# artiom-matvei/RLAO

Measured on AMD Instinct MI355X. Metric: AO env-steps/sec (batched loops), higher is better.
Workload: dtype f32; 1 GPU; 8m / 20x20 Shack-Hartmann, 256 batched envs per GPU, integrator closed loop (BASELINE.json configs[1]); envs_per_gpu=256, envs_total=256, resolution=120, n_valid_act=357, n_signal=632, layers=1, controller=leaky integrator, gain 0.5, noise=photon, parallelism=env-shards x1, all-gather of episode returns

## Files before the change

include/aoenv.h:

```cpp
#ifndef AOENV_H
#define AOENV_H

#include <stddef.h>
#include <stdint.h>

#ifdef __cplusplus
extern "C" {
#endif

#define AOENV_ABI_VERSION 7

enum { AOENV_F32 = 0, AOENV_F64 = 1 };
enum { AOENV_WFS_SH = 0, AOENV_WFS_PYRAMID = 1 };

typedef struct AoEnv AoEnv;

typedef struct AoCfg {
    int32_t abi_version;
    int32_t dtype;
    int32_t n_env;
    int32_t resolution;
    int32_t n_layer;
    int32_t layer_res;
    int32_t n_inner;
// ... 213 lines not shown
int aoenv_set_detector(AoEnv* env, const AoDetector* cfg, void* stream);

int aoenv_set_return_accumulator(AoEnv* env, void* d_return);

int aoenv_buffer(AoEnv* env, int which, void** d_ptr, size_t* bytes);
int aoenv_download(AoEnv* env, int which, void* h_dst, size_t bytes, void* stream);
int aoenv_upload_state(AoEnv* env, int which, const void* h_src, size_t bytes, void* stream);
int aoenv_get_buff(AoEnv* env, double* h_buff);
int aoenv_set_buff(AoEnv* env, const double* h_buff);

enum AoOption {
    AOENV_OPT_FAST_WFS = 0,
    AOENV_OPT_MFMA_GEMM = 1,
    AOENV_OPT_STORE_ATM_OPD = 3,
    AOENV_OPT_FUSED_TAIL = 4,
    AOENV_OPT_FUSED_STEP = 5,
    AOENV_OPT_DEFER_RING = 6,
    AOENV_OPT_COEFS_IMAGE = 7,
    AOENV_OPT_FACTORED_RECON = 8,
    AOENV_OPT_RING_LOOKAHEAD = 9,
    AOENV_OPT_FAST_TRIG = 2,
    AOENV_OPT_ENV_WIND_PIXELS = 10,
    AOENV_OPT_STEP_PAIRS = 11,
    AOENV_OPT_FORCE_PATH = 99
};
enum AoPath {
    AOENV_PATH_PHASE_DWORD = 256,
    AOENV_PATH_GENERIC = 512,
    AOENV_PATH_PYR_ROUND_ROBIN = 1024,
    AOENV_PATH_MODAL_GEMM = 2048,
    AOENV_PATH_WF_GENERAL = 8192,
    AOENV_PATH_SCI_GENERAL = 16384,
    AOENV_PATH_SH_PLAIN = 4096
};
int aoenv_set_option(AoEnv* env, int option, int value);

int aoenv_fused_step_active(AoEnv* env);

enum AoKernel {
    AOENV_K_SHIFT_GATHER = 0, AOENV_K_MT_NORMAL, AOENV_K_GEMM_RING, AOENV_K_SCATTER, AOENV_K_PHASE,
    AOENV_K_SH_SPOTS, AOENV_K_SH_CENTROID, AOENV_K_GEMM_RECON, AOENV_K_RECON_FINISH, AOENV_K_PYRAMID, AOENV_K_SH_TAIL, AOENV_K_ENV_STEP,
    AOENV_K_DETECTOR, AOENV_K_COUNT
};
int aoenv_profile(AoEnv* env, int enable);
int aoenv_profile_read(AoEnv* env, double* h_ms, int32_t* h_count, void* stream);
int aoenv_step_counters(AoEnv* env, int64_t* h_out);

int aoenv_test_normal(int device, uint32_t seed, int n, int n_calls, double* h_out);

int aoenv_test_poisson_table(uint32_t* h_out, size_t cap_words, size_t* h_words);
int aoenv_test_poisson(int device, const float* h_lambda, int n, uint64_t seed, uint32_t frame, float lmax, float* h_out);

#ifdef __cplusplus
}
#endif
#endif
```

rlao_amd/_lib.py:

```python
from __future__ import annotations

import ctypes as C
import os

_HERE = os.path.dirname(os.path.abspath(__file__))
LIB_PATH = os.environ.get("AOENV_LIB") or os.path.join(_HERE, "csrc", "libaoenv.so")

ABI_VERSION = 7
F32, F64 = 0, 1
WFS_SH, WFS_PYRAMID = 0, 1

(C_PUPIL, C_AB, C_INNER_IDX, C_OUTER_IDX, C_LAYER_WEIGHT, C_DM_GX, C_DM_GY, C_DM_MODES, C_ACT_IDX, C_WFS_AMP,
 C_SH_SUBAP_IDX, C_SH_REF, C_WFS_UNITS, C_RECON, C_PYR_MASK, C_PYR_TT, C_RECON_FACTORS) = range(17)
(B_SCREEN, B_OPD_ATM, B_COEFS, B_PHASE, B_FRAME, B_SIGNAL, B_TOTAL, B_RESIDUAL, B_WFS_MAX, B_XI, B_MT_STATE,
 B_COUNTERS, B_DM_PREV, B_COEFS_SEEN) = range(14)


(OPT_FAST_WFS, OPT_MFMA_GEMM, OPT_FAST_TRIG, OPT_STORE_ATM_OPD, OPT_FUSED_TAIL, OPT_FUSED_STEP, OPT_DEFER_RING, OPT_COEFS_IMAGE,
 OPT_FACTORED_RECON, OPT_RING_LOOKAHEAD, OPT_ENV_WIND_PIXELS, OPT_STEP_PAIRS) = range(12)
OPT_FORCE_PATH = 99
MAX_DELAY = 8
PATH_PHASE_DWORD, PATH_GENERIC, PATH_PYR_ROUND_ROBIN, PATH_MODAL_GEMM, PATH_SH_PLAIN, PATH_WF_GENERAL = 256, 512, 1024, 2048, 4096, 8192
PATH_SCI_GENERAL = 16384
SCI_LOG10 = 1
WF_RESIDUAL, WF_ATMOSPHERE = 1, 2
MAX_WF_MODES = 1024
KERNEL_NAMES = ("ring_prepare", "mt_normal", "gemm_ring", "ring_scatter", "phase", "sh_spots", "sh_centroid",
                "gemm_recon", "recon_finish", "pyramid", "sh_tail", "env_step", "detector")


class AoCfg(C.Structure):
    _fields_ = [(n, C.c_int32) for n in (
        "abi_version", "dtype", "n_env", "resolution", "n_layer", "layer_res", "n_inner", "n_outer", "n_act",
        "n_valid_act", "dm_separable", "wfs_type", "n_subap", "n_valid_subap", "n_signal", "cam_res", "n_loop",
        "max_group", "pyr_n_res", "pyr_n_theta", "pyr_centering", "pyr_norm_valid", "pyr_q_lo", "pyr_q_hi")] + [
            ("layer_res_l", C.c_int32 * 8)] + [(n, C.c_double) for n in (
            "atm_wavelength", "src_wavelength", "leak", "threshold_cog")]


class AoDetector(C.Structure):
    _fields_ = [("photon_noise", C.c_int32), ("bits", C.c_int32), ("emccd", C.c_int32), ("env_index_offset", C.c_int32),
                ("qe", C.c_double), ("dark_electrons", C.c_double), ("fwc", C.c_double), ("gain", C.c_double),
# ... 80 lines not shown
    "aoenv_policy_forward": (C.c_int, [C.c_void_p, C.c_void_p, C.c_void_p, C.c_void_p, C.c_void_p, C.c_void_p]),
    "aoenv_run_policy_rollout": (C.c_int, [C.c_void_p, C.POINTER(AoRollout), C.c_void_p, C.c_void_p, C.c_void_p, C.c_void_p, C.c_void_p,
                                           C.c_void_p, C.c_void_p, C.c_void_p]),
    "aoenv_compute_psf": (C.c_int, [C.c_void_p, C.c_int, C.c_void_p, C.c_void_p]),
    "aoenv_set_science": (C.c_int, [C.c_void_p, C.POINTER(AoScience), C.c_void_p]),
    "aoenv_science_psf": (C.c_int, [C.c_void_p, C.c_int, C.c_void_p, C.c_void_p]),
    "aoenv_set_science_accumulator": (C.c_int, [C.c_void_p, C.c_void_p, C.c_void_p, C.c_void_p]),
    "aoenv_set_detector": (C.c_int, [C.c_void_p, C.c_void_p, C.c_void_p]),
    "aoenv_set_return_accumulator": (C.c_int, [C.c_void_p, C.c_void_p]),
    "aoenv_buffer": (C.c_int, [C.c_void_p, C.c_int, C.POINTER(C.c_void_p), C.POINTER(C.c_size_t)]),
    "aoenv_download": (C.c_int, [C.c_void_p, C.c_int, C.c_void_p, C.c_size_t, C.c_void_p]),
    "aoenv_upload_state": (C.c_int, [C.c_void_p, C.c_int, C.c_void_p, C.c_size_t, C.c_void_p]),
    "aoenv_set_wind_env": (C.c_int, [C.c_void_p, C.c_void_p, C.c_int, C.c_void_p]),
    "aoenv_get_clock_env": (C.c_int, [C.c_void_p, C.c_void_p]),
    "aoenv_set_clock_env": (C.c_int, [C.c_void_p, C.c_void_p]),
    "aoenv_set_r0_env": (C.c_int, [C.c_void_p, C.c_void_p, C.c_double, C.c_void_p]),
    "aoenv_get_r0_env": (C.c_int, [C.c_void_p, C.c_void_p]),
    "aoenv_get_buff": (C.c_int, [C.c_void_p, C.c_void_p]),
    "aoenv_set_buff": (C.c_int, [C.c_void_p, C.c_void_p]),
    "aoenv_set_option": (C.c_int, [C.c_void_p, C.c_int, C.c_int]),
    "aoenv_profile": (C.c_int, [C.c_void_p, C.c_int]),
    "aoenv_profile_read": (C.c_int, [C.c_void_p, C.c_void_p, C.c_void_p, C.c_void_p]),
    "aoenv_step_counters": (C.c_int, [C.c_void_p, C.c_void_p]),
    "aoenv_test_normal": (C.c_int, [C.c_int, C.c_uint32, C.c_int, C.c_int, C.c_void_p]),
    "aoenv_test_poisson_table": (C.c_int, [C.c_void_p, C.c_size_t, C.POINTER(C.c_size_t)]),
    "aoenv_test_poisson": (C.c_int, [C.c_int, C.c_void_p, C.c_int, C.c_uint64, C.c_uint32, C.c_float, C.c_void_p]),
}


class AoEnvError(RuntimeError):
    pass


_lib = None


def load():
    global _lib
    if _lib is not None:
        return _lib
    if not os.path.exists(LIB_PATH):
        raise AoEnvError(f"{LIB_PATH} not found: build it with `python -c 'import __graft_entry__ as g; g.build()'` "
                         "(there is no CPU fallback)")
    import torch
    lib = C.CDLL(LIB_PATH)
    for name, (res, args) in EXPORTS.items():
        if name == "aoenv_step_counters" and os.environ.get("AOENV_LIB") and not hasattr(lib, name):
            continue
        fn = getattr(lib, name)
        fn.restype = res
        fn.argtypes = args
    if lib.aoenv_abi_version() != ABI_VERSION:
        raise AoEnvError(f"libaoenv ABI {lib.aoenv_abi_version()} != binding ABI {ABI_VERSION}")
    _lib = lib
    return lib


def check(rc: int):
    if rc != 0:
        raise AoEnvError(load().aoenv_last_error().decode("utf-8", "replace"))
```

rlao_amd/csrc/camera_sh6.hpp:

```cpp
#pragma once
#include "detector.hpp"
#include "sh_device.hpp"

namespace ao {

typedef float f32x16s __attribute__((ext_vector_type(16)));

__device__ inline f32x16s camera_pack(const float (&Ia)[6], const float (&Ib)[6]) {
    return f32x16s{Ia[0], Ia[1], Ia[2], Ia[3], Ib[0], Ib[1], Ib[2], Ib[3], Ia[4], Ia[5], Ib[4], Ib[5], 0.f, 0.f, 0.f, 0.f};
}
__device__ inline void camera_unpack(const f32x16s& v, float (&Ia)[6], float (&Ib)[6]) {
    Ia[0] = v[0]; Ia[1] = v[1]; Ia[2] = v[2]; Ia[3] = v[3]; Ib[0] = v[4]; Ib[1] = v[5]; Ib[2] = v[6]; Ib[3] = v[7];
    Ia[4] = v[8]; Ia[5] = v[9]; Ib[4] = v[10]; Ib[5] = v[11];
}
__device__ inline void camera_rotate(f32x16s& v) {
    v = f32x16s{v[4], v[5], v[6], v[7], v[8], v[9], v[10], v[11], v[0], v[1], v[2], v[3], 0.f, 0.f, 0.f, 0.f};
}

template <bool PHOTON_ONLY = false>
__device__ inline void camera_sh6_lane(f32x16s& pxv, bool ok, uint32_t px0, int cam, uint32_t e, const DetectorCfg& det,
                                       const uint32_t* __restrict__ tab, float lmax) {
    auto pix_of = [&](int p) {
        const int t = p >> 2, s4 = p & 3;
        return px0 + (uint32_t)((t < 2 ? s4 : 4 + (s4 & 1)) * cam + ((t == 1 || (t == 2 && s4 >= 2)) ? 3 : 0));
// ... 63 lines not shown
                                                      : poisson_ptrs(det.dark_e, word_of(o, sl4), word_of(o2, sl4), pix_of(4 * t + sl4) | 0x80000000u, e, det);
            }
            if (has_read) {
                uint32_t o[4];
                quad_bits(qid, e, det, kDrawReadout, o);
                quad_normals(o, nrm);
            }
#pragma unroll
            for (int sl4 = 0; sl4 < 4; ++sl4) pxv[sl4] = detector_finish(pxv[sl4], det, dark[sl4], nrm[sl4]);
            camera_rotate(pxv);
        }
    }
}

typedef __attribute__((address_space(1))) const void* ao_gptr_t;
typedef __attribute__((address_space(3))) void* ao_lptr_t;
__device__ inline void alias_table_to_lds(const uint32_t* __restrict__ tab, int words, uint32_t* lds, int wave, int n_waves, int lane) {
    for (int i0 = wave * 256; i0 < words; i0 += n_waves * 256) {
        const int i = i0 + 4 * lane;
        if (i < words) __builtin_amdgcn_global_load_lds((ao_gptr_t)(tab + i), (ao_lptr_t)(lds + i0), 16, 0, 0);
    }
}

}
```

rlao_amd/csrc/common.hpp:

```cpp
#pragma once
#include <hip/hip_runtime.h>
#include <stdint.h>
#include <stddef.h>

#include <string>
#include <vector>

#include "aoenv.h"

namespace ao {

constexpr int kWave = 64;
constexpr int kMaxLayer = 8;
constexpr int kMtN = 624;
constexpr int kMaxSplits = 16;
constexpr int kMaxModes = 512;

int fail(const char* fmt, ...);
#define AO_HIP(call)                                                                          \
    do {                                                                                      \
        hipError_t e_ = (call);                                                               \
        if (e_ != hipSuccess)                                                                 \
            return ::ao::fail("%s:%d: %s -> %s", __FILE__, __LINE__, #call, hipGetErrorString(e_)); \
    } while (0)
// ... 283 lines not shown
    float* wfs_max;
    const float* fac_m;
    const float* fac_m2c_t;
    const short* slot_of;
    const float* amp_pupil;
    const float* gxa;
    const float* gya;
    size_t ga_env;
    DetectorCfg det;
    PoissonAlias pa;
    const float* ring_x[kMaxLayer];
    int ring_splits[kMaxLayer];
    const int* outer_idx;
    int n_outer;
    float* next_zx[kMaxLayer];
    int next_sx[kMaxLayer], next_sy[kMaxLayer];
    const int* inner_idx;
    int n_inner, zx_ld;
    int n_modes, n_subap, n_valid, n_env;
    LayerTaps taps2[kMaxLayer];
};
int step_fused_supported(int R, int n_subap, int n_valid, int n_act, int n_modes);
int step_alias_capacity(int n_act);
int launch_env_step(const StepArgs& a, const StarEnv<float>& star, hipStream_t st);
bool env_step_pairable(const StepArgs& a, const StarEnv<float>& star);
int launch_env_step_pair(const StepArgs& a, hipStream_t st);

template <typename T>
struct RolloutActionArgs {
    const T* obs;
    T* action;
    const T* fr;
    const T* fl_t;
    const int* act_slot;
    const T* sigma_env;
    T gain, sigma;
    int n_act, n_valid_act, n_filter;
    uint32_t seed_lo, seed_hi, counter, env_offset;
};
constexpr size_t kRolloutLdsMax = 160 * 1024;
size_t rollout_action_lds(int n_valid_act, int n_filter, size_t esz);
template <typename T>
int launch_rollout_action(const RolloutActionArgs<T>& a, int n_env, hipStream_t st);

template <typename T>
struct DisturbArgs {
    const T* coefs;
    T* seen;
    const T* modes_t;
// ... 141 lines not shown
```

rlao_amd/csrc/env.hip:

```cpp
#include <algorithm>
#include <cmath>
#include <cstdarg>
#include <cstdio>
#include <cstring>
#include <initializer_list>
#include <new>
#include <utility>

#include "common.hpp"
#include "delay.hpp"
#include "dev_block.hpp"
#include "dm_tables.hpp"
#include "detector.hpp"
#include "disturb.hpp"
#include "modal.hpp"
#include "policy.hpp"
#include "sh_device.hpp"
#include "science.hpp"
#include "star_env.hpp"
#include "wavefront.hpp"

namespace ao {

static thread_local std::string g_err;
// ... 216 lines not shown
    bool act_slot_dirty = true;
    void* rollout_scratch = nullptr;
    uint32_t explore_counter = 0;
    uint64_t explore_seed = 0;
    bool explore_seeded = false;
    struct Policy {
        bool set = false, mfma = false;
        Block mem;
        int H = 0, F = 0, Kp = 0;
        double slope = 0, clamp_abs = 0, b3 = 0;
        void *w1 = nullptr, *b1 = nullptr, *w2 = nullptr, *b2 = nullptr, *w3 = nullptr, *wt1 = nullptr, *wt2 = nullptr;
        void *proj_fr = nullptr, *proj_fl_t = nullptr, *hid1 = nullptr, *hid2 = nullptr;
    } policy;
    std::vector<Block> allocs;
    bool use_fast_wfs = true;
    bool use_mfma = true;
    bool use_fast_trig = true;
    bool use_fused_tail = true;
    bool use_fused_step = true;
    bool store_opd_atm = false;
    bool atm_user_defined = false;
    int force_path = 0;
    bool use_step_pairs = true;
    struct StepPair { bool on = false; double buff2[kMaxLayer][2] = {}; } pair;
    int64_t step_launches = 0, step_covered = 0;
    bool prof_on = false;
    struct ProfEv { int stage; hipEvent_t a, b; int n; };
    std::vector<ProfEv> prof_ev;

    template <typename T> T* as(void* p_) const { return static_cast<T*>(p_); }
    void* screen_ptr(int l) const { return static_cast<char*>(screen) + layer[l].scr_off * esz; }
    void* minmax_ptr(int l) const { return static_cast<char*>(minmax) + (size_t)l * E * 2 * esz; }
    void* xbuf_ptr(int l) const { return static_cast<char*>(xbuf) + (size_t)l * kMaxSplits * E * noutmax * esz; }
    void* zx_pipe_ptr(int buf, int l) const { return static_cast<char*>(zx_pipe) + ((size_t)buf * L + l) * E * Kmax * esz; }
};

namespace {

int dmalloc(AoEnv* env, void** p, size_t bytes, bool zero = true);
static int alloc_dm_rows(AoEnv* env) {
    if (env->esz == 4 && env->nAct <= 128) {
        if (!env->dm_rows)
            AO_TRY(dmalloc(env, (void**)&env->dm_rows, (size_t)env->E * (cdiv(env->R, 128) * 128) * 4 * env->ga_stride * sizeof(float)));
    } else if (!env->coefs_img) {
        AO_TRY(dmalloc(env, &env->coefs_img, (size_t)env->E * env->nAct * env->nAct * env->esz));
    }
// ... 601 lines not shown
    if (env->det.active) env->det.frame_counter += 1;
    a.det = env->det;
    a.pa = env->alias();
    take_rings(env, a);
    const Layer& y0 = env->layer[0];
    a.outer_idx = y0.outer_idx;
    a.n_outer = y0.nout;
    a.inner_idx = y0.inner_idx;
    a.n_inner = y0.nin;
    a.zx_ld = y0.K;
    a.n_modes = env->n_modes;
    a.n_subap = env->nSub;
    a.n_valid = env->nVal;
    a.n_env = env->E;
    const bool pair = env->pair.on;
    if (pair) {
        for (int l = 0; l < env->L; ++l) {
            a.taps2[l] = a.k.pa.taps[l];
            taps_from_buff(env->pair.buff2[l], a.taps2[l]);
        }
    }
    {
        AO_PROF_N(env, ENV_STEP, st, pair ? 2 : 1);
        AO_TRY(pair ? launch_env_step_pair(a, st) : launch_env_step(a, env->star_env<float>(), st));
    }
    env->step_launches += 1;
    env->step_covered += pair ? 2 : 1;
    rings_written(env);
    if (pair) {
        for (int l = 0; l < env->L; ++l) {
            LayerClock& c = env->layer[l].clk;
            if (c.ratio[0] == 0 && c.ratio[1] == 0) continue;
            int bx, by;
            if (clock_rounds(c.ratio, 0, &bx, &by) > 0 || clock_subpixel(c.ratio, c.buff, &bx, &by))
                return fail("internal: a step covered by the launch before it crossed a pixel");
        }
        if (env->det.active) env->det.frame_counter += 1;
    }
    return 0;
}

bool step_pair_eligible(AoEnv* env) {
    if (!env->use_step_pairs || env->esz != 4 || !fused_step_ok<float>(env) || env->per_env_wind) return false;
    if (env->disturb.set || env->wf.recorded() || env->store_opd_atm) return false;
    StepArgs a{};
    a.sc = sh_const<float>(env);
    a.det = env->det;
// ... 2220 lines not shown
    if (env->per_env_wind) return fail("the shard runs per-env clocks (aoenv_set_wind_env): use aoenv_set_clock_env");
    for (int l = 0; l < env->L; ++l) {
        if (std::fabs(h_buff[2 * l]) >= 1 || std::fabs(h_buff[2 * l + 1]) >= 1) return fail("|buff| must be < 1");
        env->layer[l].clk.buff[0] = h_buff[2 * l]; env->layer[l].clk.buff[1] = h_buff[2 * l + 1];
    }
    return 0;
}

int aoenv_fused_step_active(AoEnv* env) {
    if (!env) return 0;
    return env->c.dtype == AOENV_F32 && fused_step_ok<float>(env) ? 1 : 0;
}

int aoenv_set_option(AoEnv* env, int option, int value) {
    AO_CHECK_ENV(env);
    switch (option) {
        case AOENV_OPT_FAST_WFS: env->use_fast_wfs = value != 0; return 0;
        case AOENV_OPT_MFMA_GEMM: env->use_mfma = value != 0; return 0;
        case AOENV_OPT_FAST_TRIG: env->use_fast_trig = value != 0; return 0;
        case AOENV_OPT_STORE_ATM_OPD: env->store_opd_atm = value != 0; return 0;
        case AOENV_OPT_FUSED_TAIL: env->use_fused_tail = value != 0; return 0;
        case AOENV_OPT_FUSED_STEP: env->use_fused_step = value != 0; return 0;
        case AOENV_OPT_STEP_PAIRS: env->use_step_pairs = value != 0; return 0;
        case AOENV_OPT_DEFER_RING: env->defer_ring = value != 0; return 0;
        case AOENV_OPT_FACTORED_RECON: env->use_factored_recon = value != 0; return 0;
        case AOENV_OPT_RING_LOOKAHEAD:
            if (!value)
                for (int l = 0; l < env->L; ++l) forget_lookahead(env->layer[l]);
            env->use_lookahead = value != 0;
            return 0;
        case AOENV_OPT_COEFS_IMAGE:
            if (value) AO_TRY(alloc_dm_rows(env));
            env->use_coefs_img = value != 0;
            return 0;
        case AOENV_OPT_ENV_WIND_PIXELS:
            if (value < 1 || value > 8) return fail("AOENV_OPT_ENV_WIND_PIXELS: %d outside [1, 8]", value);
            if (env->per_env_wind)
                for (int l = 0; l < env->L; ++l)
                    if (env->layer[l].env_rounds >= value)
                        return fail("AOENV_OPT_ENV_WIND_PIXELS: layer %d holds a per-env wind of %d px/frame or more, the ceiling cannot go to %d",
                                    l, env->layer[l].env_rounds, value);
            env->wind_pixels = value;
            return 0;
        case AOENV_OPT_FORCE_PATH:
            if (value & ~(AOENV_PATH_PHASE_DWORD | AOENV_PATH_GENERIC | AOENV_PATH_PYR_ROUND_ROBIN | AOENV_PATH_MODAL_GEMM | AOENV_PATH_SH_PLAIN |
                          AOENV_PATH_WF_GENERAL | AOENV_PATH_SCI_GENERAL))
// ... 1 lines not shown
            env->force_path = value;
            return 0;
        default: return fail("unknown option %d", option);
    }
}

int aoenv_profile(AoEnv* env, int enable) {
    AO_CHECK_ENV(env);
    for (auto& e : env->prof_ev) { (void)hipEventDestroy(e.a); (void)hipEventDestroy(e.b); }
    env->prof_ev.clear();
    env->prof_on = enable != 0;
    if (enable) env->step_launches = env->step_covered = 0;
    return 0;
}

int aoenv_step_counters(AoEnv* env, int64_t* h_out) {
    AO_CHECK_ENV(env);
    if (!h_out) return fail("null argument");
    h_out[0] = env->step_launches;
    h_out[1] = env->step_covered;
    return 0;
}

int aoenv_profile_read(AoEnv* env, double* h_ms, int32_t* h_count, void* stream) {
    AO_CHECK_ENV(env);
    if (!h_ms || !h_count) return fail("null argument");
    AO_HIP(hipStreamSynchronize(static_cast<hipStream_t>(stream)));
    for (int k = 0; k < AOENV_K_COUNT; ++k) { h_ms[k] = 0; h_count[k] = 0; }
    for (auto& e : env->prof_ev) {
        float ms = 0;
        AO_HIP(hipEventElapsedTime(&ms, e.a, e.b));
        h_ms[e.stage] += ms;
        h_count[e.stage] += e.n;
    }
    return 0;
}

int aoenv_test_normal(int device, uint32_t seed, int n, int n_calls, double* h_out) {
    if (n < 2 || n % 2 || n_calls < 1 || !h_out) return fail("aoenv_test_normal: bad arguments");
    DeviceGuard ao_device_guard(device);
    if (!ao_device_guard.ok) return fail("hipSetDevice(%d) failed", device);
    Block mem;
    AO_TRY(block_alloc(mem, {kMtN * 4, 4, (size_t)n * 8, 4}, false));
    uint32_t* st = static_cast<uint32_t*>(mem.part(0));
    int* pos = static_cast<int*>(mem.part(1));
    double* zx = static_cast<double*>(mem.part(2));
// ... 12 lines not shown
```

rlao_amd/csrc/step_body_text.hpp:

```cpp
    constexpr bool STAR = SPEC == STEP_STAR;
    constexpr bool GEN = SPEC == STEP_GENERAL || STAR;
    constexpr bool CAM_PHOTON_ONLY = SPEC == STEP_PHOTON;
    using namespace fstep;
    using fast6::EST;
    extern __shared__ __align__(16) unsigned char lds_raw[];
    float* lds = reinterpret_cast<float*>(lds_raw);
    const KArgs<float>& k = a.k;
    const int R = k.R, nA = k.n_act, S = k.pa.S;
    const int nAp = (nA + 3) & ~3, SS = nAp + 1;
    float* cimg = lds + L.cimg;
    float* s1 = lds + L.s1;
#if STEP_BODY_SUB != 2
    const int w_ = threadIdx.x >> 6;
#else
    const int w_ = tid2 >> 6;
#endif
    float* mapt = lds + L.mapt + w_ * (WR * WC);
    short* slot_s = reinterpret_cast<short*>(lds + L.slot);
    cplx<float>* E0 = reinterpret_cast<cplx<float>*>(lds + L.e0);
    float* sl = lds + L.sl;
    float* img_s = lds + L.img;
    const uint32_t* tab_s = reinterpret_cast<const uint32_t*>(lds + L.tab);
#if STEP_BODY_SUB != 2
    __shared__ double red[4][16];
    __shared__ double red_tail[16];
// ... 307 lines not shown
    }
    if (ok) {
        const int kk = a.sc.subap_idx[s];
        li = kk / n_sub;
        lj = kk - li * n_sub;
    }
#if STEP_BODY_SUB == 2
    DetectorCfg det2 = a.det;
    det2.frame_counter += 1u;
#define STEP_BODY_DET det2
#else
#define STEP_BODY_DET a.det
#endif
#if STEP_BODY_SUB == 1
#define STEP_BODY_STORE_FRAME false
#else
#define STEP_BODY_STORE_FRAME a.store_frame
#endif
    if (cam_active) {
        f32x16s pxv = camera_pack(Ia, Ib);
        if (cam_photons) {
            asm volatile("s_waitcnt vmcnt(0)" ::: "memory");
            lds_barrier();
        }
        camera_sh6_lane<CAM_PHOTON_ONLY>(pxv, ok, (uint32_t)((li * 6) * R + lj * 6 + q3), R, (uint32_t)e, STEP_BODY_DET, tab_s, a.pa.lmax);
        camera_unpack(pxv, Ia, Ib);
    }
    if (ok) {
        if (STEP_BODY_STORE_FRAME) {
            float* fr = a.frame + pix0 + (size_t)(li * 6) * R + lj * 6 + q3;
#pragma unroll
            for (int u = 0; u < 6; ++u) {
                fr[(size_t)u * R] = Ia[u];
                fr[(size_t)u * R + 3] = Ib[u];
            }
        }
#pragma unroll
        for (int u = 0; u < 6; ++u) {
            mx = Ia[u] > mx ? Ia[u] : mx;
            mx = Ib[u] > mx ? Ib[u] : mx;
        }
    }
    if ((GEN || SPEC == STEP_CAMERA) && STEP_BODY_STORE_FRAME && cam_active && (a.det.dark_e > 0.f || a.det.readout_noise != 0.f)) {
#if STEP_BODY_SUB != 2
        const float rtab = recip_table_lane();
#else
        const float rtab = 1.0f / (float)(lane + 1);
#endif
        for (int idx = tid; idx < n_sub * n_sub * 9; idx += 1024) {
            const int kk = idx / 9, j = idx - 9 * kk;
            if (slot_s[kk] < 0) {
                const int i2 = kk / n_sub, j2 = kk - i2 * n_sub;
                uint32_t pix[4];
                sh6_quad_pixels(j, i2 * 6, j2 * 6, R, pix);
                f32x4d v = {0.f, 0.f, 0.f, 0.f};
                detector_quad<false>(v, pix, pix[0], (uint32_t)e, STEP_BODY_DET, rtab, a.pa);
#pragma unroll
                for (int s4 = 0; s4 < 4; ++s4) a.frame[pix0 + pix[s4]] = v[s4];
            }
        }
    }
    int late0;
    asm volatile("v_mov_b32 %0, 0" : "=v"(late0) : "v"(mx));
    const int n_sig = 2 * n_valid, n4 = n_sig / 4, A = k.n_valid_act;
    const int km = tid >> 4, l16 = tid & 15;
    f32x4s mv[10];
    if (4 * w < a.n_modes) {
        const f32x4s* row = reinterpret_cast<const f32x4s*>(a.fac_m + (size_t)(km < a.n_modes ? km : 0) * n_sig);
#pragma unroll
        for (int j = 0; j < 10; ++j) mv[j] = row[(l16 + 16 * j < n4 ? l16 + 16 * j : 0) + late0];
    } else {
#pragma unroll
        for (int j = 0; j < 10; ++j) mv[j] = f32x4s{0.f, 0.f, 0.f, 0.f};
    }
    const float ref0 = a.sc.ref[ok ? s : 0], ref1 = a.sc.ref[ok ? n_valid + s : 0];
#if STEP_BODY_SUB == 2
    float act_prev = carry_o, dm_prev_c = carry_cn;
    if (false) {
#else
    float act_prev = 0.f, dm_prev_c = 0.f;
    if (a.fa.do_integrate) {
#endif
        const size_t io = (size_t)e * (nA * nA) + (has_act ? act_px : 0) + late0;
        act_prev = (a.fa.gain_from_obs != 0.f) ? a.fa.obs[io] : a.fa.action[io];
        dm_prev_c = a.fa.dm_prev[(size_t)e * k.n_valid_act + (has_act ? tid : 0) + late0];
    }
    for (int off = 32; off > 0; off >>= 1) {
        const float o = __shfl_down(mx, off);
        mx = o > mx ? o : mx;
    }
    if (lane == 0) red_mx[w] = mx;
    lds_barrier();
    mx = red_mx[0];
#pragma unroll
    for (int q = 1; q < 16; ++q) mx = red_mx[q] > mx ? red_mx[q] : mx;
    if (tid == 0) a.wfs_max[e] = mx;
    for (int i = tid; i < nA * nA; i += 1024) img_s[i] = 0.f;
    float cut;
    if constexpr (STAR) cut = (star.thr ? star.thr[e] : a.sc.threshold) * mx;
    else cut = a.sc.threshold * mx;
    {
        float norm = 0.f, m0 = 0.f, m1 = 0.f;
#pragma unroll
        for (int u = 0; u < 6; ++u) {
            const float xa = Ia[u] < cut ? 0.f : Ia[u], xb = Ib[u] < cut ? 0.f : Ib[u];
            const float rs = xa + xb;
            norm += rs;
            m0 += rs * (float)u;
            m1 += xa * (float)q3 + xb * (float)(q3 + 3);
        }
        norm += __shfl_down(norm, 1) + __shfl_down(norm, 2);
        m0 += __shfl_down(m0, 1) + __shfl_down(m0, 2);
        m1 += __shfl_down(m1, 1) + __shfl_down(m1, 2);
        if (ok && q3 == 0) {
            float c0 = 0.f, c1 = 0.f;
            if (norm != 0.f) {
                c0 = m0 / norm;
                c1 = m1 / norm;
            }
            const float v0 = (c0 - ref0) / a.sc.units, v1 = (c1 - ref1) / a.sc.units;
            sl[s] = v0;
            sl[n_valid + s] = v1;
            a.signal[(size_t)e * 2 * n_valid + s] = v0;
            a.signal[(size_t)e * 2 * n_valid + n_valid + s] = v1;
        }
    }
    lds_barrier();

    const int img = nA * nA;
    float* tm = img_s + img;
    {
        const f32x4s* s4 = reinterpret_cast<const f32x4s*>(sl);
        float acc = 0.f;
#pragma unroll
        for (int j = 0; j < 10; ++j) {
            const bool okj = l16 + 16 * j < n4;
            const f32x4s sv = s4[okj ? l16 + 16 * j : 0];
#if STEP_BODY_SUB == 0
            const float d = ((mv[j][0] * sv[0] + mv[j][1] * sv[1]) + mv[j][2] * sv[2]) + mv[j][3] * sv[3];
#else
            const float d = __builtin_fmaf(mv[j][3], sv[3], __builtin_fmaf(mv[j][2], sv[2], __builtin_fmaf(mv[j][0], sv[0], mv[j][1] * sv[1])));
#endif
            acc += okj ? d : 0.f;
        }
#pragma unroll
        for (int off = 8; off > 0; off >>= 1) acc += __shfl_xor(acc, off, 16);
        if (km < a.n_modes && l16 == 0) tm[km] = acc;
    }
    const int n_grp = (A + 3) / 4, g = tid >> 2, part = tid & 3;
    const bool g_ok = g < n_grp;
    f32x4s cv[13];
    int late1;
    asm volatile("v_mov_b32 %0, 0" : "=v"(late1) : "v"(late0));
    if (16 * w < n_grp) {
#pragma unroll
        for (int j = 0; j < 13; ++j)
            __builtin_memcpy(&cv[j], a.fac_m2c_t + (part + 4 * j < a.n_modes ? (size_t)(part + 4 * j) * A + 4 * (g_ok ? g : 0) : 0) + late1, 16);
    } else {
#pragma unroll
        for (int j = 0; j < 13; ++j) cv[j] = f32x4s{0.f, 0.f, 0.f, 0.f};
    }
    lds_barrier();
    double ss = 0.0;
    {
        float acc[4] = {0.f, 0.f, 0.f, 0.f};
#pragma unroll
        for (int j = 0; j < 13; ++j) {
            const bool okj = part + 4 * j < a.n_modes;
            const float t = tm[okj ? part + 4 * j : 0];
#pragma unroll
            for (int d = 0; d < 4; ++d) acc[d] += okj ? cv[j][d] * t : 0.f;
        }
#pragma unroll
        for (int d = 0; d < 4; ++d) {
            acc[d] += __shfl_xor(acc[d], 1, 4);
            acc[d] += __shfl_xor(acc[d], 2, 4);
        }
        if (has_act) {
            const float mine = part == 0 ? acc[0] : (part == 1 ? acc[1] : (part == 2 ? acc[2] : acc[3]));
            if (a.fa.do_integrate) {
                const float act = (a.fa.gain_from_obs != 0.f) ? a.fa.gain_from_obs * act_prev : act_prev;
#if STEP_BODY_SUB == 0
                const float cn = dm_prev_c * a.fa.leak + act * 1e-6f;
#else
                const float cn = __builtin_fmaf(dm_prev_c, a.fa.leak, act * 1e-6f);
// ... 41 lines not shown
```

rlao_amd/csrc/step_kernel.hip:

```cpp
#include "step_kernel.hpp"

#include "sh_device.hpp"

namespace ao {

static StepLds step_lds_layout(int n_act, int n_subap, int n_valid, int n_modes) {
    using namespace fstep;
    StepLds L;
    const int nAp = (n_act + 3) & ~3, SS = nAp + 1;
    int o = 0;
    auto take = [&](int words) { const int at = o; o += (words + 3) & ~3; return at; };
    const int sl_words = (2 * n_valid + 3) & ~3, img_words = n_act * n_act + n_modes;
    L.cimg = take(n_act * n_act);
    L.s1 = take(2 * PR * SS);
    L.mapt = take(16 * WR * WC);
    L.tab = L.cimg;
    L.tab_cap = o - L.tab;
    L.slot = take((n_subap * n_subap + 1) / 2);
    L.e0 = take(std::max(2 * n_valid * fast6::EST, sl_words + img_words));
    L.sl = L.e0;
    L.img = L.e0 + sl_words;
    L.total = o;
    return L;
}

int step_fused_supported(int R, int n_subap, int n_valid, int n_act, int n_modes) {
    if (R % n_subap || R / n_subap != fast6::P) return 0;
    if (R > fstep::TX || R % 4) return 0;
    if (n_valid > 16 * 21 || n_subap * n_subap > 32767 || n_act > 32) return 0;
    if (n_modes < 1 || n_modes > 52 || (2 * n_valid) % 4 != 0 || 2 * n_valid > 640) return 0;
    const StepLds L = step_lds_layout(n_act, n_subap, n_valid, n_modes);
    return (size_t)L.total * 4 <= 160 * 1024 - 1024 ? 1 : 0;
}

int step_alias_capacity(int n_act) { return step_lds_layout(n_act, 1, 1, 1).tab_cap; }

static StepSpec step_spec(const StepArgs& a, const StarEnv<float>& star) {
    if (star.amp || star.thr) return STEP_STAR;
    if (!a.sc.fast_trig || a.sc.plain) return STEP_GENERAL;
    if (!a.det.active) return STEP_NOCAM;
    const DetectorCfg& d = a.det;
    const bool after_photons = d.dark_e > 0.f || d.readout_noise != 0.f || d.qe != 1.f || d.gain != 1.f || d.fwc > 0.f || d.bits > 0;
    return d.photon_noise && !after_photons ? STEP_PHOTON : STEP_CAMERA;
}

static int step_tables_fit(const StepArgs& a, const StepLds& L) {
    if (a.det.active && a.det.photon_noise && (!a.pa.tab || a.pa.words > L.tab_cap || a.pa.lmax < palias::kCoarseStep))
        return fail("fused step: the photon-noise tables are missing or do not fit (%d words, room for %d)", a.pa.words, L.tab_cap);
    return 0;
}

int launch_env_step(const StepArgs& a, const StarEnv<float>& star, hipStream_t st) {
    const StepLds L = step_lds_layout(a.k.n_act, a.n_subap, a.n_valid, a.n_modes);
    AO_TRY(step_tables_fit(a, L));
    switch (step_spec(a, star)) {
        case STEP_STAR: return launch_env_step_spec<STEP_STAR>(a, L, star, st);
        case STEP_GENERAL: return launch_env_step_spec<STEP_GENERAL>(a, L, star, st);
        case STEP_NOCAM: return launch_env_step_spec<STEP_NOCAM>(a, L, star, st);
        case STEP_PHOTON: return launch_env_step_spec<STEP_PHOTON>(a, L, star, st);
        default: return launch_env_step_spec<STEP_CAMERA>(a, L, star, st);
    }
}

bool env_step_pairable(const StepArgs& a, const StarEnv<float>& star) {
    const StepSpec s = step_spec(a, star);
    if (a.k.pa.env_taps != nullptr) return false;
    return s == STEP_PHOTON || (s == STEP_CAMERA && a.det.bits > 0 && a.det.bits <= 21);
}

int launch_env_step_pair(const StepArgs& a, hipStream_t st) {
    const StepLds L = step_lds_layout(a.k.n_act, a.n_subap, a.n_valid, a.n_modes);
    const StarEnv<float> star{nullptr, nullptr};
    if (!env_step_pairable(a, star)) return fail("internal: a step pair on a launch that has no pair kernel");
    if (!a.fa.do_integrate || a.fa.gain_from_obs == 0.f) return fail("internal: a step pair without the on-device integrator");
    AO_TRY(step_tables_fit(a, L));
    switch (step_spec(a, star)) {
        case STEP_PHOTON: return launch_env_step_pair_spec<STEP_PHOTON>(a, L, star, st);
        default: return launch_env_step_pair_spec<STEP_CAMERA>(a, L, star, st);
    }
}

}
```

rlao_amd/csrc/step_kernel.hpp:

```cpp
#pragma once
#include "common.hpp"

namespace ao {

enum StepSpec {
    STEP_GENERAL = 0,
    STEP_NOCAM = 1,
    STEP_PHOTON = 2,
    STEP_CAMERA = 3,
    STEP_STAR = 4
};

namespace fstep {
constexpr int TX = 128, PR = 64;
constexpr int WR = 16 + 3, WC = 32 + 4;
constexpr int WC4 = WC / 4;
constexpr int NV4 = (WR * WC4 + 63) / 64;
}

struct StepLds {
    int cimg, s1, mapt, slot, e0, sl, img, total;
    int tab, tab_cap;
};

template <int SPEC>
int launch_env_step_spec(const StepArgs& a, const StepLds& L, const StarEnv<float>& star, hipStream_t st);
extern template int launch_env_step_spec<STEP_GENERAL>(const StepArgs&, const StepLds&, const StarEnv<float>&, hipStream_t);
extern template int launch_env_step_spec<STEP_NOCAM>(const StepArgs&, const StepLds&, const StarEnv<float>&, hipStream_t);
extern template int launch_env_step_spec<STEP_PHOTON>(const StepArgs&, const StepLds&, const StarEnv<float>&, hipStream_t);
extern template int launch_env_step_spec<STEP_CAMERA>(const StepArgs&, const StepLds&, const StarEnv<float>&, hipStream_t);
extern template int launch_env_step_spec<STEP_STAR>(const StepArgs&, const StepLds&, const StarEnv<float>&, hipStream_t);

template <int SPEC>
int launch_env_step_pair_spec(const StepArgs& a, const StepLds& L, const StarEnv<float>& star, hipStream_t st);
extern template int launch_env_step_pair_spec<STEP_PHOTON>(const StepArgs&, const StepLds&, const StarEnv<float>&, hipStream_t);
extern template int launch_env_step_pair_spec<STEP_CAMERA>(const StepArgs&, const StepLds&, const StarEnv<float>&, hipStream_t);

}
```

rlao_amd/env.py:

```python
from __future__ import annotations

import ctypes as C
import os
from collections import namedtuple
from types import SimpleNamespace

import numpy as np

from . import _lib as L
from . import calib

_NP_DT = {"f32": np.float32, "f64": np.float64}
CAMERAS = {
    "ideal": ({}, {}),
    "papyrus": ({}, dict(photonNoise=True)),
    "razor": (dict(sensor="CMOS", FWC=10000, bits=10, QE=0.56, darkCurrent=5, integrationTime="samplingTime"),
              dict(photonNoise=True, readoutNoise=14)),
}


def _torch():
    import torch
    return torch

# ... 452 lines not shown
        return out

    def upload_state(self, which: int, arr, stream=0, dtype=None):
        a = np.ascontiguousarray(arr, dtype=self.np_dtype if dtype is None else dtype)
        L.check(self.lib.aoenv_upload_state(self.h, which, a.ctypes.data_as(C.c_void_p), a.nbytes, C.c_void_p(stream)))

    def profile(self, enable: bool):
        L.check(self.lib.aoenv_profile(self.h, int(enable)))

    def profile_read(self, stream=0) -> dict:
        n = len(L.KERNEL_NAMES)
        ms = np.zeros(n)
        cnt = np.zeros(n, dtype=np.int32)
        L.check(self.lib.aoenv_profile_read(self.h, ms.ctypes.data_as(C.c_void_p), cnt.ctypes.data_as(C.c_void_p),
                                            C.c_void_p(stream)))
        return {k: (float(ms[i]), int(cnt[i])) for i, k in enumerate(L.KERNEL_NAMES)}

    def step_counters(self) -> tuple:
        if not hasattr(self.lib, "aoenv_step_counters"):
            raise L.AoEnvError("the library loaded through AOENV_LIB was built before aoenv_step_counters")
        out = np.zeros(2, dtype=np.int64)
        L.check(self.lib.aoenv_step_counters(self.h, out.ctypes.data_as(C.c_void_p)))
        return int(out[0]), int(out[1])

    def get_buff(self, n_layer: int) -> np.ndarray:
        out = np.zeros((max(n_layer, 1), 2))
        L.check(self.lib.aoenv_get_buff(self.h, out.ctypes.data_as(C.c_void_p)))
        return out[:n_layer]

    def set_buff(self, buff):
        b = np.ascontiguousarray(buff, dtype=np.float64)
        L.check(self.lib.aoenv_set_buff(self.h, b.ctypes.data_as(C.c_void_p)))

    def set_wind_env(self, ratio: np.ndarray, reset_buff: bool, stream=0):
        r = np.ascontiguousarray(ratio, dtype=np.float64)
        L.check(self.lib.aoenv_set_wind_env(self.h, r.ctypes.data_as(C.c_void_p), int(reset_buff), C.c_void_p(stream)))

    def get_clock_env(self, n_layer: int, n_env: int) -> np.ndarray:
        out = np.zeros((n_layer, n_env, 4))
        L.check(self.lib.aoenv_get_clock_env(self.h, out.ctypes.data_as(C.c_void_p)))
        return out

    def set_clock_env(self, clock):
        c = np.ascontiguousarray(clock, dtype=np.float64)
        L.check(self.lib.aoenv_set_clock_env(self.h, c.ctypes.data_as(C.c_void_p)))

# ... 1481 lines not shown
```

Before: 5.848 million env-steps/s.

## Stage reconstructor factor matrices into LDS during photon wait in fused step

In the photon and camera variants of the fused step kernel, the modal factor matrices (fac_m rows and fac_m2c_t) are copied into otherwise unused LDS with global_load_lds_dwordx4. The copy is issued right after the camera-photon barrier so it overlaps the camera and centroid work. The tail then reads these matrices from LDS instead of from global memory, cutting global traffic on the latency-critical tail. It adds a waitcnt before each use, an M0-register asm dance, and a layout planner. It also adds an option and a query API, both on by default.

```diff
diff --git a/include/aoenv.h b/include/aoenv.h
--- a/include/aoenv.h
+++ b/include/aoenv.h
@@ -259,6 +259,7 @@
     AOENV_OPT_FAST_TRIG = 2,
     AOENV_OPT_ENV_WIND_PIXELS = 10,
     AOENV_OPT_STEP_PAIRS = 11,
+    AOENV_OPT_TAIL_LDS = 12,
     AOENV_OPT_FORCE_PATH = 99
 };
 enum AoPath {
@@ -283,6 +284,8 @@
 int aoenv_profile_read(AoEnv* env, double* h_ms, int32_t* h_count, void* stream);
 int aoenv_step_counters(AoEnv* env, int64_t* h_out);
 
+int aoenv_step_tail_plan(AoEnv* env, int32_t* out);
+
 int aoenv_test_normal(int device, uint32_t seed, int n, int n_calls, double* h_out);
 
 int aoenv_test_poisson_table(uint32_t* h_out, size_t cap_words, size_t* h_words);
diff --git a/rlao_amd/_lib.py b/rlao_amd/_lib.py
--- a/rlao_amd/_lib.py
+++ b/rlao_amd/_lib.py
@@ -17,7 +17,7 @@
 
 
 (OPT_FAST_WFS, OPT_MFMA_GEMM, OPT_FAST_TRIG, OPT_STORE_ATM_OPD, OPT_FUSED_TAIL, OPT_FUSED_STEP, OPT_DEFER_RING, OPT_COEFS_IMAGE,
- OPT_FACTORED_RECON, OPT_RING_LOOKAHEAD, OPT_ENV_WIND_PIXELS, OPT_STEP_PAIRS) = range(12)
+ OPT_FACTORED_RECON, OPT_RING_LOOKAHEAD, OPT_ENV_WIND_PIXELS, OPT_STEP_PAIRS, OPT_TAIL_LDS) = range(13)
 OPT_FORCE_PATH = 99
 MAX_DELAY = 8
 PATH_PHASE_DWORD, PATH_GENERIC, PATH_PYR_ROUND_ROBIN, PATH_MODAL_GEMM, PATH_SH_PLAIN, PATH_WF_GENERAL = 256, 512, 1024, 2048, 4096, 8192
@@ -144,6 +144,7 @@
     "aoenv_profile": (C.c_int, [C.c_void_p, C.c_int]),
     "aoenv_profile_read": (C.c_int, [C.c_void_p, C.c_void_p, C.c_void_p, C.c_void_p]),
     "aoenv_step_counters": (C.c_int, [C.c_void_p, C.c_void_p]),
+    "aoenv_step_tail_plan": (C.c_int, [C.c_void_p, C.c_void_p]),
     "aoenv_test_normal": (C.c_int, [C.c_int, C.c_uint32, C.c_int, C.c_int, C.c_void_p]),
     "aoenv_test_poisson_table": (C.c_int, [C.c_void_p, C.c_size_t, C.POINTER(C.c_size_t)]),
     "aoenv_test_poisson": (C.c_int, [C.c_int, C.c_void_p, C.c_int, C.c_uint64, C.c_uint32, C.c_float, C.c_void_p]),
@@ -167,7 +168,7 @@
     import torch
     lib = C.CDLL(LIB_PATH)
     for name, (res, args) in EXPORTS.items():
-        if name == "aoenv_step_counters" and os.environ.get("AOENV_LIB") and not hasattr(lib, name):
+        if name in ("aoenv_step_counters", "aoenv_step_tail_plan") and os.environ.get("AOENV_LIB") and not hasattr(lib, name):
             continue
         fn = getattr(lib, name)
         fn.restype = res
diff --git a/rlao_amd/csrc/camera_sh6.hpp b/rlao_amd/csrc/camera_sh6.hpp
--- a/rlao_amd/csrc/camera_sh6.hpp
+++ b/rlao_amd/csrc/camera_sh6.hpp
@@ -109,4 +109,26 @@
     }
 }
 
+__device__ inline void direct_load16(const float* src, const float* lds_wave_base) {
+    const uint32_t base = __builtin_amdgcn_readfirstlane((uint32_t)(uintptr_t)(ao_lptr_t)lds_wave_base);
+    uint32_t m0_was;
+    asm volatile("s_mov_b32 %0, m0\n\ts_mov_b32 m0, %2\n\ts_nop 0\n\tglobal_load_lds_dwordx4 %1, off\n\ts_mov_b32 m0, %0"
+                 : "=&s"(m0_was) : "v"(src), "s"(base) : "memory");
 }
+__device__ inline void rows_to_lds(const float* __restrict__ src, int src_stride, int n_rows, float* lds, int lds_stride, uint32_t lds_magic, int wave,
+                                   int n_waves, int lane) {
+    const int words = n_rows * lds_stride;
+    for (int i0 = wave * 256; i0 < words; i0 += n_waves * 256) {
+        const int i = i0 + 4 * lane;
+        const int r = (int)__umulhi((uint32_t)i, lds_magic), c = i - r * lds_stride;
+        if (i < words) direct_load16(src + r * src_stride + c, lds + i0);
+    }
+}
+__device__ inline void run_to_lds(const float* __restrict__ src, int words, float* lds, int wave, int n_waves, int lane) {
+    for (int i0 = wave * 256; i0 < words; i0 += n_waves * 256) {
+        const int i = i0 + 4 * lane;
+        if (i < words) direct_load16(src + i, lds + i0);
+    }
+}
+
+}
diff --git a/rlao_amd/csrc/common.hpp b/rlao_amd/csrc/common.hpp
--- a/rlao_amd/csrc/common.hpp
+++ b/rlao_amd/csrc/common.hpp
@@ -329,9 +329,10 @@
 };
 int step_fused_supported(int R, int n_subap, int n_valid, int n_act, int n_modes);
 int step_alias_capacity(int n_act);
-int launch_env_step(const StepArgs& a, const StarEnv<float>& star, hipStream_t st);
+int launch_env_step(const StepArgs& a, const StarEnv<float>& star, bool tail_lds, hipStream_t st);
 bool env_step_pairable(const StepArgs& a, const StarEnv<float>& star);
-int launch_env_step_pair(const StepArgs& a, hipStream_t st);
+int launch_env_step_pair(const StepArgs& a, bool tail_lds, hipStream_t st);
+void step_tail_plan_query(const StepArgs& a, const StarEnv<float>& star, bool tail_lds, int32_t out[4]);
 
 template <typename T>
 struct RolloutActionArgs {
diff --git a/rlao_amd/csrc/env.hip b/rlao_amd/csrc/env.hip
--- a/rlao_amd/csrc/env.hip
+++ b/rlao_amd/csrc/env.hip
@@ -262,6 +262,7 @@
     bool atm_user_defined = false;
     int force_path = 0;
     bool use_step_pairs = true;
+    bool use_tail_lds = true;
     struct StepPair { bool on = false; double buff2[kMaxLayer][2] = {}; } pair;
     int64_t step_launches = 0, step_covered = 0;
     bool prof_on = false;
@@ -909,7 +910,7 @@
     }
     {
         AO_PROF_N(env, ENV_STEP, st, pair ? 2 : 1);
-        AO_TRY(pair ? launch_env_step_pair(a, st) : launch_env_step(a, env->star_env<float>(), st));
+        AO_TRY(pair ? launch_env_step_pair(a, env->use_tail_lds, st) : launch_env_step(a, env->star_env<float>(), env->use_tail_lds, st));
     }
     env->step_launches += 1;
     env->step_covered += pair ? 2 : 1;
@@ -3176,6 +3177,7 @@
         case AOENV_OPT_FUSED_TAIL: env->use_fused_tail = value != 0; return 0;
         case AOENV_OPT_FUSED_STEP: env->use_fused_step = value != 0; return 0;
         case AOENV_OPT_STEP_PAIRS: env->use_step_pairs = value != 0; return 0;
+        case AOENV_OPT_TAIL_LDS: env->use_tail_lds = value != 0; return 0;
         case AOENV_OPT_DEFER_RING: env->defer_ring = value != 0; return 0;
         case AOENV_OPT_FACTORED_RECON: env->use_factored_recon = value != 0; return 0;
         case AOENV_OPT_RING_LOOKAHEAD:
@@ -3223,6 +3225,23 @@
     return 0;
 }
 
+int aoenv_step_tail_plan(AoEnv* env, int32_t* out) {
+    AO_CHECK_ENV(env);
+    if (!out) return fail("null argument");
+    out[0] = out[1] = out[2] = out[3] = 0;
+    if (env->esz != 4 || !fused_step_ok<float>(env)) return 0;
+    StepArgs a{};
+    a.sc = sh_const<float>(env);
+    a.det = env->det;
+    a.k.n_act = env->nAct;
+    a.k.n_valid_act = env->A;
+    a.n_subap = env->nSub;
+    a.n_valid = env->nVal;
+    a.n_modes = env->n_modes;
+    step_tail_plan_query(a, env->star_env<float>(), env->use_tail_lds, out);
+    return 0;
+}
+
 int aoenv_profile_read(AoEnv* env, double* h_ms, int32_t* h_count, void* stream) {
     AO_CHECK_ENV(env);
     if (!h_ms || !h_count) return fail("null argument");
diff --git a/rlao_amd/csrc/step_body_text.hpp b/rlao_amd/csrc/step_body_text.hpp
--- a/rlao_amd/csrc/step_body_text.hpp
+++ b/rlao_amd/csrc/step_body_text.hpp
@@ -1,6 +1,7 @@
     constexpr bool STAR = SPEC == STEP_STAR;
     constexpr bool GEN = SPEC == STEP_GENERAL || STAR;
     constexpr bool CAM_PHOTON_ONLY = SPEC == STEP_PHOTON;
+    constexpr bool TAIL_LDS = SPEC == STEP_PHOTON || SPEC == STEP_CAMERA;
     using namespace fstep;
     using fast6::EST;
     extern __shared__ __align__(16) unsigned char lds_raw[];
@@ -354,6 +355,10 @@
         if (cam_photons) {
             asm volatile("s_waitcnt vmcnt(0)" ::: "memory");
             lds_barrier();
+            if constexpr (TAIL_LDS) {
+                if (L.m2c_off >= 0) rows_to_lds(a.fac_m2c_t, k.n_valid_act, a.n_modes, lds + L.m2c_off, L.m2c_stride, L.m2c_magic, w, 16, lane);
+                if (L.m_rows > 0) run_to_lds(a.fac_m, L.m_rows * 2 * n_valid, lds + L.m_off, w, 16, lane);
+            }
         }
         camera_sh6_lane<CAM_PHOTON_ONLY>(pxv, ok, (uint32_t)((li * 6) * R + lj * 6 + q3), R, (uint32_t)e, STEP_BODY_DET, tab_s, a.pa.lmax);
         camera_unpack(pxv, Ia, Ib);
@@ -397,7 +402,8 @@
     const int n_sig = 2 * n_valid, n4 = n_sig / 4, A = k.n_valid_act;
     const int km = tid >> 4, l16 = tid & 15;
     f32x4s mv[10];
-    if (4 * w < a.n_modes) {
+    const bool mv_lds = TAIL_LDS && 4 * w + 4 <= L.m_rows;
+    if (!mv_lds && 4 * w < a.n_modes) {
         const f32x4s* row = reinterpret_cast<const f32x4s*>(a.fac_m + (size_t)(km < a.n_modes ? km : 0) * n_sig);
 #pragma unroll
         for (int j = 0; j < 10; ++j) mv[j] = row[(l16 + 16 * j < n4 ? l16 + 16 * j : 0) + late0];
@@ -444,6 +450,9 @@
         norm += __shfl_down(norm, 1) + __shfl_down(norm, 2);
         m0 += __shfl_down(m0, 1) + __shfl_down(m0, 2);
         m1 += __shfl_down(m1, 1) + __shfl_down(m1, 2);
+        if constexpr (TAIL_LDS) {
+            if (L.m_rows > 0) asm volatile("s_waitcnt vmcnt(0)" ::: "memory");
+        }
         if (ok && q3 == 0) {
             float c0 = 0.f, c1 = 0.f;
             if (norm != 0.f) {
@@ -461,6 +470,11 @@
 
     const int img = nA * nA;
     float* tm = img_s + img;
+    if (TAIL_LDS && 4 * w + 4 <= L.m_rows) {
+        const f32x4s* row = reinterpret_cast<const f32x4s*>(lds + L.m_off + km * n_sig + late0);
+#pragma unroll
+        for (int j = 0; j < 10; ++j) mv[j] = row[l16 + 16 * j < n4 ? l16 + 16 * j : 0];
+    }
     {
         const f32x4s* s4 = reinterpret_cast<const f32x4s*>(sl);
         float acc = 0.f;
@@ -484,7 +498,8 @@
     f32x4s cv[13];
     int late1;
     asm volatile("v_mov_b32 %0, 0" : "=v"(late1) : "v"(late0));
-    if (16 * w < n_grp) {
+    const bool cv_lds = TAIL_LDS && L.m2c_off >= 0;
+    if (!cv_lds && 16 * w < n_grp) {
 #pragma unroll
         for (int j = 0; j < 13; ++j)
             __builtin_memcpy(&cv[j], a.fac_m2c_t + (part + 4 * j < a.n_modes ? (size_t)(part + 4 * j) * A + 4 * (g_ok ? g : 0) : 0) + late1, 16);
@@ -492,7 +507,15 @@
 #pragma unroll
         for (int j = 0; j < 13; ++j) cv[j] = f32x4s{0.f, 0.f, 0.f, 0.f};
     }
-    lds_barrier();
+    if constexpr (TAIL_LDS) {
+        if (cv_lds) asm volatile("s_waitcnt vmcnt(0)" ::: "memory");
+    }
+    lds_barrier();
+    if (cv_lds && 16 * w < n_grp) {
+        const float* c0 = lds + L.m2c_off + 4 * (g_ok ? g : 0) + late1;
+#pragma unroll
+        for (int j = 0; j < 13; ++j) cv[j] = *reinterpret_cast<const f32x4s*>(c0 + (part + 4 * j < a.n_modes ? (part + 4 * j) * L.m2c_stride : 0));
+    }
     double ss = 0.0;
     {
         float acc[4] = {0.f, 0.f, 0.f, 0.f};
diff --git a/rlao_amd/csrc/step_kernel.hip b/rlao_amd/csrc/step_kernel.hip
--- a/rlao_amd/csrc/step_kernel.hip
+++ b/rlao_amd/csrc/step_kernel.hip
@@ -3,26 +3,6 @@
 #include "sh_device.hpp"
 
 namespace ao {
-
-static StepLds step_lds_layout(int n_act, int n_subap, int n_valid, int n_modes) {
-    using namespace fstep;
-    StepLds L;
-    const int nAp = (n_act + 3) & ~3, SS = nAp + 1;
-    int o = 0;
-    auto take = [&](int words) { const int at = o; o += (words + 3) & ~3; return at; };
-    const int sl_words = (2 * n_valid + 3) & ~3, img_words = n_act * n_act + n_modes;
-    L.cimg = take(n_act * n_act);
-    L.s1 = take(2 * PR * SS);
-    L.mapt = take(16 * WR * WC);
-    L.tab = L.cimg;
-    L.tab_cap = o - L.tab;
-    L.slot = take((n_subap * n_subap + 1) / 2);
-    L.e0 = take(std::max(2 * n_valid * fast6::EST, sl_words + img_words));
-    L.sl = L.e0;
-    L.img = L.e0 + sl_words;
-    L.total = o;
-    return L;
-}
 
 int step_fused_supported(int R, int n_subap, int n_valid, int n_act, int n_modes) {
     if (R % n_subap || R / n_subap != fast6::P) return 0;
@@ -50,8 +30,23 @@
     return 0;
 }
 
-int launch_env_step(const StepArgs& a, const StarEnv<float>& star, hipStream_t st) {
-    const StepLds L = step_lds_layout(a.k.n_act, a.n_subap, a.n_valid, a.n_modes);
+static StepLds step_launch_layout(const StepArgs& a, const StarEnv<float>& star, bool tail_lds) {
+    const StepSpec s = step_spec(a, star);
+    const bool stage = tail_lds && (s == STEP_PHOTON || s == STEP_CAMERA);
+    return step_tail_plan(a.k.n_act, a.n_subap, a.n_valid, a.k.n_valid_act, a.n_modes, a.det.active && a.det.photon_noise, stage);
+}
+
+void step_tail_plan_query(const StepArgs& a, const StarEnv<float>& star, bool tail_lds, int32_t out[4]) {
+    const StepLds L = step_launch_layout(a, star, tail_lds);
+    const int words = (L.m2c_off >= 0 ? a.n_modes * L.m2c_stride : 0) + L.m_rows * 2 * a.n_valid;
+    out[0] = L.m2c_off >= 0 ? 1 : 0;
+    out[1] = L.m_rows;
+    out[2] = words > 0 ? 1 : 0;
+    out[3] = words;
+}
+
+int launch_env_step(const StepArgs& a, const StarEnv<float>& star, bool tail_lds, hipStream_t st) {
+    const StepLds L = step_launch_layout(a, star, tail_lds);
     AO_TRY(step_tables_fit(a, L));
     switch (step_spec(a, star)) {
         case STEP_STAR: return launch_env_step_spec<STEP_STAR>(a, L, star, st);
@@ -68,9 +63,9 @@
     return s == STEP_PHOTON || (s == STEP_CAMERA && a.det.bits > 0 && a.det.bits <= 21);
 }
 
-int launch_env_step_pair(const StepArgs& a, hipStream_t st) {
-    const StepLds L = step_lds_layout(a.k.n_act, a.n_subap, a.n_valid, a.n_modes);
+int launch_env_step_pair(const StepArgs& a, bool tail_lds, hipStream_t st) {
     const StarEnv<float> star{nullptr, nullptr};
+    const StepLds L = step_launch_layout(a, star, tail_lds);
     if (!env_step_pairable(a, star)) return fail("internal: a step pair on a launch that has no pair kernel");
     if (!a.fa.do_integrate || a.fa.gain_from_obs == 0.f) return fail("internal: a step pair without the on-device integrator");
     AO_TRY(step_tables_fit(a, L));
diff --git a/rlao_amd/csrc/step_kernel.hpp b/rlao_amd/csrc/step_kernel.hpp
--- a/rlao_amd/csrc/step_kernel.hpp
+++ b/rlao_amd/csrc/step_kernel.hpp
@@ -1,5 +1,6 @@
 #pragma once
 #include "common.hpp"
+#include "sh_device.hpp"
 
 namespace ao {
 
@@ -21,7 +22,60 @@
 struct StepLds {
     int cimg, s1, mapt, slot, e0, sl, img, total;
     int tab, tab_cap;
+    int m2c_off, m2c_stride, m_off, m_rows;
+    unsigned m2c_magic;
 };
+
+inline StepLds step_lds_layout(int n_act, int n_subap, int n_valid, int n_modes) {
+    using namespace fstep;
+    StepLds L;
+    const int nAp = (n_act + 3) & ~3, SS = nAp + 1;
+    int o = 0;
+    auto take = [&](int words) { const int at = o; o += (words + 3) & ~3; return at; };
+    const int sl_words = (2 * n_valid + 3) & ~3, img_words = n_act * n_act + n_modes;
+    L.cimg = take(n_act * n_act);
+    L.s1 = take(2 * PR * SS);
+    L.mapt = take(16 * WR * WC);
+    L.tab = L.cimg;
+    L.tab_cap = o - L.tab;
+    L.slot = take((n_subap * n_subap + 1) / 2);
+    L.e0 = take(std::max(2 * n_valid * fast6::EST, sl_words + img_words));
+    L.sl = L.e0;
+    L.img = L.e0 + sl_words;
+    L.total = o;
+    L.m2c_off = -1;
+    L.m2c_stride = L.m_off = L.m_rows = 0;
+    L.m2c_magic = 0;
+    return L;
+}
+
+#ifndef AOENV_TAIL_M_FIRST
+#define AOENV_TAIL_M_FIRST 0
+#endif
+inline StepLds step_tail_plan(int n_act, int n_subap, int n_valid, int n_valid_act, int n_modes, bool photons, bool stage = true) {
+    StepLds L = step_lds_layout(n_act, n_subap, n_valid, n_modes);
+    if (!photons || !stage) return L;
+    const int n_sig = 2 * n_valid;
+    int at = L.img + ((n_act * n_act + n_modes + 3) & ~3);
+    const int end = L.total;
+    auto take_m2c = [&] {
+        const int stride = (n_valid_act + 3) & ~3;
+        if (at + n_modes * stride > end) return;
+        L.m2c_off = at;
+        L.m2c_stride = stride;
+        L.m2c_magic = (unsigned)((1ull << 32) / (unsigned)stride + 1);
+        at += n_modes * stride;
+    };
+    auto take_m = [&] {
+        const int fit = at < end ? (end - at) / n_sig : 0;
+        L.m_rows = (fit < n_modes ? fit : n_modes) & ~3;
+        L.m_off = at;
+        at += L.m_rows * n_sig;
+    };
+    if (AOENV_TAIL_M_FIRST) { take_m(); take_m2c(); }
+    else { take_m2c(); take_m(); }
+    return L;
+}
 
 template <int SPEC>
 int launch_env_step_spec(const StepArgs& a, const StepLds& L, const StarEnv<float>& star, hipStream_t st);
diff --git a/rlao_amd/env.py b/rlao_amd/env.py
--- a/rlao_amd/env.py
+++ b/rlao_amd/env.py
@@ -498,6 +498,13 @@
         out = np.zeros(2, dtype=np.int64)
         L.check(self.lib.aoenv_step_counters(self.h, out.ctypes.data_as(C.c_void_p)))
         return int(out[0]), int(out[1])
+
+    def tail_plan(self) -> dict:
+        if not hasattr(self.lib, "aoenv_step_tail_plan"):
+            raise L.AoEnvError("the library loaded through AOENV_LIB was built before aoenv_step_tail_plan")
+        out = np.zeros(4, dtype=np.int32)
+        L.check(self.lib.aoenv_step_tail_plan(self.h, out.ctypes.data_as(C.c_void_p)))
+        return {"m2c": bool(out[0]), "m_rows": int(out[1]), "region": int(out[2]), "words": int(out[3])}
 
     def get_buff(self, n_layer: int) -> np.ndarray:
         out = np.zeros((max(n_layer, 1), 2))
```

Measured after the change: 5.673 million env-steps/s. -3.0%, worse.
